# IamArmanNikkhah/viewport-entropy-toolkit

Hardware: NVIDIA B200
Metric: user-frame samples/sec (bin+weighted entropy, 200 tiles) (higher is better)
Workload: dtype f64

## Files before the change

### include/vet_b200.h

```cpp
#ifndef VET_B200_H
#define VET_B200_H

#include <stdint.h>

#ifdef __cplusplus
extern "C" {
#endif

typedef struct vet_handle vet_handle;

typedef enum {
  VET_OK = 0,
  VET_ERR_INVALID_ARG = -1,
  VET_ERR_CUDA = -2,
  VET_ERR_UNSUPPORTED = -3,
  VET_ERR_NOMEM = -4
} vet_status;

enum { VET_F32 = 0, VET_F64 = 1 };
enum { VET_TRANSITION_LITERAL = 0, VET_TRANSITION_TEXTBOOK = 1 };
enum { VET_MISSING = 0xFFFF };

enum {
  VET_FLAG_OUT_OF_RANGE = 1,
  VET_FLAG_EMPTY_FRAME = 2,
  VET_FLAG_NO_COMMON_USER = 4
};

typedef struct {
  int32_t device;
  int32_t video_width;
  int32_t video_height;
  int32_t num_tile_counts;
  const int32_t* tile_counts;
  double fov_angle;
  double power_factor;
  int32_t use_weight_distribution;
  const double* const* centres;
  const double* lon_by_px;
  const double* lat_by_py;
  const int32_t* num_tiles;
  int32_t naive_tile_width;
  int32_t naive_tile_height;
  int32_t regime;
} vet_config;

enum { VET_REGIME_AUTO = 0, VET_REGIME_DIRECT = 1 };

const char* vet_last_error(void);
const char* vet_version(void);

#define VET_I8_MIN_FRAMES 384
enum {
  VET_OPT_WEIGHTED_KERNEL = 0,
  VET_OPT_STREAM_KERNEL = 1,
  VET_OPT_TRANSITION_KERNEL = 2,
  VET_OPT_CLUSTER_TAIL = 3,
  VET_OPT_T3_PAIR_SCRATCH = 4,
  VET_OPT_T3_ASSUME_MISSING = 5,
  VET_OPT_ANALYZE_OVERLAP = 6,
  VET_OPT_HOST_BATCH_FRAMES = 7,
  VET_OPT_T4_LIST_CAP = 8,
  VET_OPT_CUDA_GRAPH = 9,
  VET_OPT_HOST_LAYOUT = 10,
  VET_OPT_COUNT = 11
};
int vet_set_option(vet_handle* h, int option, int value);
int vet_get_option(const vet_handle* h, int option, int* value);

int vet_create(vet_handle** out, const vet_config* cfg);
int vet_destroy(vet_handle* h);

int vet_num_tiles(const vet_handle* h, int k);
int64_t vet_num_cells(const vet_handle* h);

int vet_lattice(const vet_handle* h, int k, double* centres_host);
int vet_cell_lut(const vet_handle* h, int k, uint16_t* lut_host);

int vet_decode(vet_handle* h, const void* packed_dev, int dtype, int64_t n, double* vec_dev,
               int32_t* cell_dev, void* stream);

int vet_nearest_tile(vet_handle* h, int k, const double* vec_dev, int64_t n, int32_t* idx_dev,
                     void* stream);

int vet_tile_weights(vet_handle* h, int k, const double* vec_dev, int64_t n, double* w_dev,
                     void* stream);

int vet_angular_distances(vet_handle* h, int k, const double* vec_dev, int64_t n, double* d_dev,
                          void* stream);

int vet_vector_angles(vet_handle* h, const double* a_dev, const double* b_dev, int64_t n, double* d_dev,
                      void* stream);

int vet_spatial_vectors(vet_handle* h, const double* vec_dev, int64_t F, int64_t U,
                        double* entropy_dev, double* per_k_dev, double* hist0_dev,
                        uint16_t* assign0_dev, void* stream);

int vet_transition_vectors(vet_handle* h, const double* vec_dev, int64_t F, int64_t U,
                           double* entropy_dev, double* per_k_dev, int32_t* prev_count0_dev,
                           uint16_t* pairs0_dev, int mode, void* stream);

int vet_spatial(vet_handle* h, const void* packed_dev, int dtype, int64_t F, int64_t U,
                double* entropy_dev, double* per_k_dev, double* hist0_dev, uint16_t* assign0_dev,
                void* stream);

int vet_transition(vet_handle* h, const void* packed_dev, int dtype, int64_t F, int64_t U,
                   double* entropy_dev, double* per_k_dev, int32_t* prev_count0_dev,
                   uint16_t* pairs0_dev, int mode, void* stream);

int vet_analyze(vet_handle* h, const void* packed_dev, int dtype, int64_t F, int64_t U,
                double* sp_entropy_dev, double* sp_per_k_dev, double* hist0_dev, uint16_t* assign0_dev,
                double* tr_entropy_dev, double* tr_per_k_dev, int32_t* prev_count0_dev,
                uint16_t* pairs0_dev, int mode, void* stream);

int vet_spatial_host(vet_handle* h, const void* packed_host, int dtype, int64_t F, int64_t U,
                     double* entropy_host, double* per_k_host, double* hist0_host,
                     uint16_t* assign0_host);
int vet_transition_host(vet_handle* h, const void* packed_host, int dtype, int64_t F, int64_t U,
                        double* entropy_host, double* per_k_host, int32_t* prev_count0_host,
                        uint16_t* pairs0_host, int mode);
int vet_analyze_host(vet_handle* h, const void* packed_host, int dtype, int64_t F, int64_t U,
                     double* sp_entropy_host, double* sp_per_k_host, double* hist0_host, uint16_t* assign0_host,
                     double* tr_entropy_host, double* tr_per_k_host, int32_t* prev_count0_host,
                     uint16_t* pairs0_host, int mode);

int vet_users_accumulate(vet_handle* h, const void* packed_dev, int dtype, int64_t F, int64_t U,
                         int64_t total_frames, int64_t* acc_dev, void* stream);
int vet_users_finish(vet_handle* h, const int64_t* acc_dev, int64_t U, int64_t total_frames,
                     double* entropy_dev, double* per_k_dev, double* hist0_dev, void* stream);

int vet_naive_points(vet_handle* h, const double* lonlat_dev, int64_t F, int64_t U, int32_t tile_width,
                     int32_t tile_height, int32_t use_weight_distribution, double* entropy_dev,
                     int32_t* lon_idx_dev, int32_t* lat_idx_dev, void* stream);

int vet_poll_flags(vet_handle* h, void* stream, uint32_t* flags);

int64_t vet_launch_count(const vet_handle* h);
int64_t vet_graph_replays(const vet_handle* h);

enum {
  VET_KERNEL_STREAM = 0,
  VET_KERNEL_EPILOGUE = 1,
  VET_KERNEL_TRANSITION = 2,
  VET_KERNEL_TRANSITION_TAIL = 3,
  VET_KERNEL_COUNT = 4
};
int vet_profile_enable(vet_handle* h, int on);
int vet_profile_read(vet_handle* h, double* ms_by_kernel, int64_t* launches_by_kernel);

#ifdef __cplusplus
}
#endif
#endif
```

### viewport_entropy_toolkit_b200/_native.py

```python
from __future__ import annotations

import ctypes as C
import os
from pathlib import Path
from typing import Optional

LIB_PATH = Path(__file__).resolve().parent / "_lib" / "libvet_b200.so"

VET_OK = 0
VET_ERR_INVALID_ARG = -1
VET_ERR_CUDA = -2
VET_ERR_UNSUPPORTED = -3
VET_ERR_NOMEM = -4

VET_F32, VET_F64 = 0, 1
VET_TRANSITION_LITERAL, VET_TRANSITION_TEXTBOOK = 0, 1
VET_MISSING = 0xFFFF
VET_FLAG_OUT_OF_RANGE, VET_FLAG_EMPTY_FRAME, VET_FLAG_NO_COMMON_USER = 1, 2, 4
VET_REGIME_AUTO, VET_REGIME_DIRECT = 0, 1
I8_MIN_FRAMES = 384

OPTIONS = {
    "weighted_kernel": (0, {"auto": 0, "fp64": 1, "i8": 2}),
    "stream_kernel": (1, {"auto": 0, "simple": 1, "cells": 2, "global": 3}),
    "transition_kernel": (2, {"auto": 0, "v1": 1, "v2": 2, "v3": 3}),
    "cluster_tail": (3, {"off": 0, "auto": 1, "force": 2}),
    "t3_pair_scratch": (4, {"off": 0, "on": 1}),
    "t3_assume_missing": (5, {"off": 0, "on": 1}),
    "analyze_overlap": (6, {"off": 0, "on": 1}),
    "host_batch_frames": (7, {"auto": 0}),
    "t4_list_cap": (8, {"auto": 0}),
    "cuda_graph": (9, {"off": 0, "on": 1}),
    "host_layout": (10, {"tuv": 0, "uv": 1}),
}


class VetConfig(C.Structure):
    _fields_ = [
        ("device", C.c_int32),
        ("video_width", C.c_int32),
        ("video_height", C.c_int32),
        ("num_tile_counts", C.c_int32),
        ("tile_counts", C.POINTER(C.c_int32)),
        ("fov_angle", C.c_double),
        ("power_factor", C.c_double),
        ("use_weight_distribution", C.c_int32),
        ("centres", C.POINTER(C.POINTER(C.c_double))),
        ("lon_by_px", C.POINTER(C.c_double)),
        ("lat_by_py", C.POINTER(C.c_double)),
        ("num_tiles", C.POINTER(C.c_int32)),
        ("naive_tile_width", C.c_int32),
        ("naive_tile_height", C.c_int32),
        ("regime", C.c_int32),
    ]


_P = C.c_void_p
_I64 = C.c_int64
SYMBOLS = {
    "vet_last_error": (C.c_char_p, []),
    "vet_version": (C.c_char_p, []),
    "vet_set_option": (C.c_int, [_P, C.c_int, C.c_int]),
    "vet_get_option": (C.c_int, [_P, C.c_int, C.POINTER(C.c_int)]),
    "vet_create": (C.c_int, [C.POINTER(_P), C.POINTER(VetConfig)]),
    "vet_destroy": (C.c_int, [_P]),
    "vet_num_tiles": (C.c_int, [_P, C.c_int]),
    "vet_num_cells": (_I64, [_P]),
    "vet_lattice": (C.c_int, [_P, C.c_int, _P]),
    "vet_cell_lut": (C.c_int, [_P, C.c_int, _P]),
    "vet_decode": (C.c_int, [_P, _P, C.c_int, _I64, _P, _P, _P]),
    "vet_nearest_tile": (C.c_int, [_P, C.c_int, _P, _I64, _P, _P]),
    "vet_tile_weights": (C.c_int, [_P, C.c_int, _P, _I64, _P, _P]),
    "vet_angular_distances": (C.c_int, [_P, C.c_int, _P, _I64, _P, _P]),
    "vet_vector_angles": (C.c_int, [_P, _P, _P, _I64, _P, _P]),
    "vet_spatial_vectors": (C.c_int, [_P, _P, _I64, _I64, _P, _P, _P, _P, _P]),
    "vet_transition_vectors": (C.c_int, [_P, _P, _I64, _I64, _P, _P, _P, _P, C.c_int, _P]),
    "vet_spatial": (C.c_int, [_P, _P, C.c_int, _I64, _I64, _P, _P, _P, _P, _P]),
    "vet_transition": (C.c_int, [_P, _P, C.c_int, _I64, _I64, _P, _P, _P, _P, C.c_int, _P]),
    "vet_analyze": (C.c_int, [_P, _P, C.c_int, _I64, _I64, _P, _P, _P, _P, _P, _P, _P, _P, C.c_int, _P]),
    "vet_spatial_host": (C.c_int, [_P, _P, C.c_int, _I64, _I64, _P, _P, _P, _P]),
    "vet_transition_host": (C.c_int, [_P, _P, C.c_int, _I64, _I64, _P, _P, _P, _P, C.c_int]),
    "vet_analyze_host": (C.c_int, [_P, _P, C.c_int, _I64, _I64, _P, _P, _P, _P, _P, _P, _P, _P, C.c_int]),
    "vet_users_accumulate": (C.c_int, [_P, _P, C.c_int, _I64, _I64, _I64, _P, _P]),
    "vet_users_finish": (C.c_int, [_P, _P, _I64, _I64, _P, _P, _P, _P]),
    "vet_naive_points": (C.c_int, [_P, _P, _I64, _I64, C.c_int32, C.c_int32, C.c_int32, _P, _P, _P, _P]),
    "vet_poll_flags": (C.c_int, [_P, _P, C.POINTER(C.c_uint32)]),
    "vet_launch_count": (_I64, [_P]),
    "vet_graph_replays": (_I64, [_P]),
    "vet_profile_enable": (C.c_int, [_P, C.c_int]),
    "vet_profile_read": (C.c_int, [_P, C.POINTER(C.c_double), C.POINTER(C.c_int64)]),
}
KERNEL_NAMES = ("stream", "epilogue", "transition", "transition_tail")

_lib: Optional[C.CDLL] = None


class NativeLibraryError(RuntimeError):
    """The CUDA library is missing or incomplete (build it with
    `python __graft_entry__.py`)."""


def load_library() -> C.CDLL:
    global _lib
    if _lib is not None:
        return _lib
    path = Path(os.environ.get("VET_B200_LIB", LIB_PATH))
    if not path.exists():
        raise NativeLibraryError(
            f"{path} not found: the CUDA extension is not built (run `python __graft_entry__.py`); "
            "there is no CPU fallback")
    lib = C.CDLL(str(path))
    for name, (restype, argtypes) in SYMBOLS.items():
        try:
            fn = getattr(lib, name)
        except AttributeError as e:
            raise NativeLibraryError(f"{path} does not export {name}") from e
        fn.restype = restype
        fn.argtypes = argtypes
    _lib = lib
    return lib


def last_error() -> str:
    return load_library().vet_last_error().decode("utf-8", "replace")
```

### viewport_entropy_toolkit_b200/csrc/vet_whist_i8.cuh

```cuda
#pragma once
#include <cuda.h>

#include "vet_common.cuh"
#include "vet_stream_tma.cuh"

namespace vet {

constexpr int kI8Slices = 5;
constexpr int kI8FracBits = 39;
constexpr int kI8TilesPerBlock = 48;
constexpr int kI8N = kI8Slices * kI8TilesPerBlock;
constexpr int kI8M = 128;
constexpr int kI8BK = 128;
constexpr int kI8Stages = 3;
constexpr int kI8StagesOne = 4;
constexpr int kI8ABytes = kI8M * kI8BK;
constexpr int kI8BBytes = kI8N * kI8BK;
constexpr int kI8StageBytes = 2 * kI8ABytes + kI8BBytes;
constexpr int kI8Threads = 192;
constexpr int kI8MaxSplit = 8;
constexpr int kI8TmemCols = 512;
constexpr int kI8SmemBytes = kI8Stages * kI8StageBytes + 1024;
static_assert(kI8StageBytes % 1024 == 0 && (kI8ABytes + kI8BBytes) % 1024 == 0, "stages must keep the 1024 B swizzle alignment");
static_assert(kI8StagesOne * (kI8ABytes + kI8BBytes) <= kI8Stages * kI8StageBytes, "both layouts share one ring");

__device__ __forceinline__ void tma_load_2d(uint32_t dst, const void* tmap, uint32_t bar, int c0, int c1) {
  asm volatile(
      "cp.async.bulk.tensor.2d.shared::cluster.global.mbarrier::complete_tx::bytes [%0], [%1, {%3, %4}], [%2];" ::"r"(dst),
      "l"(tmap), "r"(bar), "r"(c0), "r"(c1)
      : "memory");
}
__device__ __forceinline__ void tc_fence_before() { asm volatile("tcgen05.fence::before_thread_sync;" ::: "memory"); }
__device__ __forceinline__ void tc_fence_after() { asm volatile("tcgen05.fence::after_thread_sync;" ::: "memory"); }
__device__ __forceinline__ void tc_alloc(uint32_t smem_dst, uint32_t cols) {
  asm volatile("tcgen05.alloc.cta_group::1.sync.aligned.shared::cta.b32 [%0], %1;" ::"r"(smem_dst), "r"(cols) : "memory");
  asm volatile("tcgen05.relinquish_alloc_permit.cta_group::1.sync.aligned;" ::: "memory");
}
__device__ __forceinline__ void tc_dealloc(uint32_t taddr, uint32_t cols) {
  asm volatile("tcgen05.dealloc.cta_group::1.sync.aligned.b32 %0, %1;" ::"r"(taddr), "r"(cols) : "memory");
}
__device__ __forceinline__ void tc_commit(uint32_t bar) {
  asm volatile("tcgen05.commit.cta_group::1.mbarrier::arrive::one.shared::cluster.b64 [%0];" ::"r"(bar) : "memory");
}
__device__ __forceinline__ void tc_mma_i8(uint32_t d, uint64_t adesc, uint64_t bdesc, uint32_t idesc, uint32_t accumulate) {
  asm volatile(
      "{\n"
      ".reg .pred p;\n"
      "setp.ne.b32 p, %4, 0;\n"
      "tcgen05.mma.cta_group::1.kind::i8 [%0], %1, %2, %3, p;\n"
      "}\n" ::"r"(d),
      "l"(adesc), "l"(bdesc), "r"(idesc), "r"(accumulate)
      : "memory");
}
__device__ __forceinline__ void tc_ld16(uint32_t taddr, uint32_t (&r)[16]) {
  asm volatile(
      "tcgen05.ld.sync.aligned.32x32b.x16.b32 {%0, %1, %2, %3, %4, %5, %6, %7, %8, %9, %10, %11, %12, %13, %14, %15}, [%16];"
      : "=r"(r[0]), "=r"(r[1]), "=r"(r[2]), "=r"(r[3]), "=r"(r[4]), "=r"(r[5]), "=r"(r[6]), "=r"(r[7]), "=r"(r[8]), "=r"(r[9]),
        "=r"(r[10]), "=r"(r[11]), "=r"(r[12]), "=r"(r[13]), "=r"(r[14]), "=r"(r[15])
      : "r"(taddr)
      : "memory");
}
__device__ __forceinline__ void tc_wait_ld() { asm volatile("tcgen05.wait::ld.sync.aligned;" ::: "memory"); }

__device__ __forceinline__ uint64_t i8_smem_desc(uint32_t saddr) {
  return (uint64_t)((saddr & 0x3FFFFu) >> 4) | (1ull << 16) | ((uint64_t)(1024 >> 4) << 32) | (1ull << 46) | (2ull << 61);
}
constexpr uint32_t kI8InstrDesc = (2u << 4) | ((uint32_t)(kI8N >> 3) << 17) | ((uint32_t)(kI8M >> 4) << 24);

struct WhistI8Args {
  int64_t F;
  int T;
  int n_blocks;
  int row_a;
  int row_b;
  const uint32_t* flag_b;
  const uint32_t* run_if;
  int shift;
  int accumulate;
  const int2* kb_range;
  double* hist;
  int ksplit;
  int* part;
};

__global__ void __launch_bounds__(kI8Threads, 1)
k_whist_i8(const __grid_constant__ CUtensorMap tm_cnt, const __grid_constant__ CUtensorMap tm_w, WhistI8Args a) {
  const int tile_id = blockIdx.x / a.ksplit;
  const int sp = blockIdx.x % a.ksplit;
  const int nb = tile_id % a.n_blocks;
  const int mb = tile_id / a.n_blocks;
  if (a.run_if && a.run_if[mb] == 0u) return;
  extern __shared__ unsigned char smem_dyn[];
  __shared__ __align__(8) unsigned long long s_full[kI8StagesOne], s_empty[kI8StagesOne], s_accum;
  __shared__ uint32_t s_tmem;
  const int warp = threadIdx.x >> 5, lane = threadIdx.x & 31;
  const uint32_t ring = (smem_u32(smem_dyn) + 1023u) & ~1023u;
  int2 kr = a.kb_range[nb];
  if (a.ksplit > 1) {
    const int per = (kr.y - kr.x + a.ksplit - 1) / a.ksplit;
    kr.x = min(kr.y, kr.x + sp * per);
    kr.y = min(kr.y, kr.x + per);
  }
  const bool two = a.flag_b && a.flag_b[mb] != 0u;

  const uint32_t nstages = two ? kI8Stages : kI8StagesOne;
  const uint32_t stage_bytes = two ? (uint32_t)kI8StageBytes : (uint32_t)(kI8ABytes + kI8BBytes);
  const uint32_t w_off = two ? 2u * kI8ABytes : (uint32_t)kI8ABytes;
  if (threadIdx.x == 0) {
    for (int i = 0; i < kI8StagesOne; ++i) {
      mbar_init(smem_u32(&s_full[i]), 1);
      mbar_init(smem_u32(&s_empty[i]), 1);
    }
    mbar_init(smem_u32(&s_accum), 1);
    asm volatile("fence.mbarrier_init.release.cluster;" ::: "memory");
  }
  if (warp == 1) tc_alloc(smem_u32(&s_tmem), kI8TmemCols);
  tc_fence_before();
  __syncthreads();
  tc_fence_after();
  const uint32_t tmem = s_tmem;

  if (warp == 0) {
    if (lane == 0) {
      uint32_t stage = 0, phase = 0;
      for (int kb = kr.x; kb < kr.y; ++kb) {
        mbar_wait(smem_u32(&s_empty[stage]), phase ^ 1u);
        const uint32_t bar = smem_u32(&s_full[stage]);
        const uint32_t base = ring + stage * stage_bytes;
        mbar_expect_tx(bar, stage_bytes);
        tma_load_2d(base, &tm_cnt, bar, kb * kI8BK, a.row_a + mb * kI8M);
        if (two) tma_load_2d(base + kI8ABytes, &tm_cnt, bar, kb * kI8BK, a.row_b + mb * kI8M);
        tma_load_2d(base + w_off, &tm_w, bar, kb * kI8BK, nb * kI8N);
        if (++stage == nstages) {
          stage = 0;
          phase ^= 1u;
        }
      }
    }
  } else if (warp == 1) {
    if (lane == 0) {
      uint32_t stage = 0, phase = 0;
      for (int kb = kr.x; kb < kr.y; ++kb) {
        mbar_wait(smem_u32(&s_full[stage]), phase);
        tc_fence_after();
        const uint32_t base = ring + stage * stage_bytes;
#pragma unroll
        for (int k = 0; k < kI8BK / 32; ++k) {
          const uint32_t acc = (kb > kr.x || k > 0) ? 1u : 0u;
          const uint64_t bdesc = i8_smem_desc(base + w_off + k * 32);
          tc_mma_i8(tmem, i8_smem_desc(base + k * 32), bdesc, kI8InstrDesc, acc);
          if (two) tc_mma_i8(tmem + 256, i8_smem_desc(base + kI8ABytes + k * 32), bdesc, kI8InstrDesc, acc);
        }
        tc_commit(smem_u32(&s_empty[stage]));
        if (++stage == nstages) {
          stage = 0;
          phase ^= 1u;
        }
      }
      tc_commit(smem_u32(&s_accum));
    }
    __syncwarp();
  } else {
    const int q = warp & 3;
    const int64_t f = (int64_t)mb * kI8M + q * 32 + lane;
    const uint32_t lane_base = tmem + ((uint32_t)(q * 32) << 16);
    if (a.ksplit > 1) {
      int* __restrict__ part = a.part + ((int64_t)tile_id * a.ksplit + sp) * (2 * kI8N * kI8M) + q * 32 + lane;
      const bool have = kr.y > kr.x;
      if (have) {
        mbar_wait(smem_u32(&s_accum), 0u);
        tc_fence_after();
      }
#pragma unroll 1
      for (int c0 = 0; c0 < kI8N; c0 += 16) {
        uint32_t r0[16], r1[16];
#pragma unroll
        for (int j = 0; j < 16; ++j) r0[j] = r1[j] = 0u;
        if (have) {
          tc_ld16(lane_base + c0, r0);
          if (two) tc_ld16(lane_base + 256 + c0, r1);
          tc_wait_ld();
        }
#pragma unroll
        for (int j = 0; j < 16; ++j) {
          __stcg(part + (c0 + j) * kI8M, (int)r0[j]);
          if (two) __stcg(part + (kI8N + c0 + j) * kI8M, (int)r1[j]);
        }
      }
    } else {
      mbar_wait(smem_u32(&s_accum), 0u);
      tc_fence_after();
#pragma unroll 1
      for (int j0 = 0; j0 < kI8TilesPerBlock; j0 += 16) {
        double v[16];
#pragma unroll
        for (int j = 0; j < 16; ++j) v[j] = 0.0;
#pragma unroll
        for (int s = kI8Slices - 1; s >= 0; --s) {
          uint32_t r0[16], r1[16];
          tc_ld16(lane_base + s * kI8TilesPerBlock + j0, r0);
          if (two) tc_ld16(lane_base + 256 + s * kI8TilesPerBlock + j0, r1);
          tc_wait_ld();
          const double scale = __longlong_as_double((long long)(1023 + 8 * s - kI8FracBits + a.shift) << 52);
#pragma unroll
          for (int j = 0; j < 16; ++j) {
            long long x = (long long)(int)r0[j];
            if (two) x += (long long)(int)r1[j] << 8;
            v[j] = fma((double)x, scale, v[j]);
          }
        }
        if (f < a.F) {
          double* __restrict__ row = a.hist + f * (int64_t)a.T;
#pragma unroll
          for (int j = 0; j < 16; ++j) {
            const int tile = nb * kI8TilesPerBlock + j0 + j;
            if (tile < a.T) row[tile] = a.accumulate ? row[tile] + v[j] : v[j];
          }
        }
      }
    }
  }
  tc_fence_before();
  __syncthreads();
  if (warp == 1) tc_dealloc(tmem, kI8TmemCols);
}

__global__ void __launch_bounds__(kI8M) k_whist_i8_finish(WhistI8Args a) {
  const int tile_id = blockIdx.y;
  const int nb = tile_id % a.n_blocks;
  const int mb = tile_id / a.n_blocks;
  if (a.run_if && a.run_if[mb] == 0u) return;
  const int j = blockIdx.x;
  const int tile = nb * kI8TilesPerBlock + j;
  const int64_t f = (int64_t)mb * kI8M + threadIdx.x;
  if (tile >= a.T || f >= a.F) return;
  const bool two = a.flag_b && a.flag_b[mb] != 0u;
  const int* __restrict__ part = a.part + (int64_t)tile_id * a.ksplit * (2 * kI8N * kI8M) + threadIdx.x;
  int x0[kI8Slices], x1[kI8Slices];
#pragma unroll
  for (int s = 0; s < kI8Slices; ++s) x0[s] = x1[s] = 0;
#pragma unroll
  for (int sp = 0; sp < kI8MaxSplit; ++sp) {
    if (sp < a.ksplit) {
#pragma unroll
      for (int s = 0; s < kI8Slices; ++s) {
        const int* p = part + (int64_t)sp * (2 * kI8N * kI8M) + (s * kI8TilesPerBlock + j) * kI8M;
        x0[s] += __ldcg(p);
        if (two) x1[s] += __ldcg(p + kI8N * kI8M);
      }
    }
  }
  double v = 0.0;
#pragma unroll
  for (int s = kI8Slices - 1; s >= 0; --s) {
    long long x = (long long)x0[s];
    if (two) x += (long long)x1[s] << 8;
    const double scale = __longlong_as_double((long long)(1023 + 8 * s - kI8FracBits + a.shift) << 52);
    v = fma((double)x, scale, v);
  }
  double* __restrict__ row = a.hist + f * (int64_t)a.T;
  row[tile] = a.accumulate ? row[tile] + v : v;
}

struct CntPlanesArgs {
  const uint32_t* cnt;
  int64_t F;
  int cpad;
  int kp;
  int64_t plane_stride;
  uint8_t* planes;
  uint8_t* dirty;
  uint32_t* hi1;
  uint32_t* hi2;
};

__global__ void __launch_bounds__(256) k_cnt_planes(CntPlanesArgs a) {
  const int lane = threadIdx.x & 31;
  const int64_t warp = (blockIdx.x * (int64_t)blockDim.x + threadIdx.x) >> 5;
  const int64_t nwarps = ((int64_t)gridDim.x * blockDim.x) >> 5;
  const int upr = a.kp >> 7;
  const int64_t units = a.F * upr;
  uint32_t* __restrict__ p0 = reinterpret_cast<uint32_t*>(a.planes);
  uint32_t* __restrict__ p1 = reinterpret_cast<uint32_t*>(a.planes + a.plane_stride);
  uint32_t* __restrict__ p2 = reinterpret_cast<uint32_t*>(a.planes + 2 * a.plane_stride);
  constexpr int kUnroll = 4;
  for (int64_t u0 = warp * kUnroll; u0 < units; u0 += nwarps * kUnroll) {
    uint4 v[kUnroll];
#pragma unroll
    for (int i = 0; i < kUnroll; ++i) {
      const int64_t u = u0 + i;
      v[i] = make_uint4(0u, 0u, 0u, 0u);
      if (u < units) {
        const int64_t f = u / upr;
        const int c = (int)(u % upr) * 128 + lane * 4;
        if (c < a.cpad) v[i] = __ldg(reinterpret_cast<const uint4*>(a.cnt + f * (int64_t)a.cpad + c));
      }
    }
#pragma unroll
    for (int i = 0; i < kUnroll; ++i) {
      const int64_t u = u0 + i;
      if (u < units) {
        const int64_t f = u / upr;
        const int64_t o = (f * (int64_t)a.kp + (u % upr) * 128) / 4 + lane;
        const uint32_t w1 = pack_bytes(v[i], 8), w2 = pack_bytes(v[i], 16);
        p0[o] = pack_bytes(v[i], 0);
        p1[o] = w1;
        p2[o] = w2;
        if (w1 && *reinterpret_cast<volatile uint32_t*>(&a.hi1[f >> 7]) == 0u) atomicOr(&a.hi1[f >> 7], 1u);
        if (w2 && *reinterpret_cast<volatile uint32_t*>(&a.hi2[f >> 7]) == 0u) atomicOr(&a.hi2[f >> 7], 1u);
        if (u % upr == 0 && lane == 0) a.dirty[f] = 3;
      }
    }
  }
}

}
```

Measured before the change: 418.2 billion.

## Restructure i8 weighted-histogram kernel with per-block k-lists, variable N, in-kernel third plane

Replaces the contiguous per-block k-range with an explicit list of k-blocks per tile block, makes the MMA N width and tiles-per-block runtime values, and interleaves slices per tile in the TMEM column layout. The third count plane (high bits) is now handled by a second sweep inside the same kernel, with a drain barrier to reuse TMEM, instead of a separate accumulate launch. The run_if early exit is removed. This aims to skip empty k-blocks and cut launches and hist read-modify-write passes, at the cost of a more complex barrier protocol and extra partial-buffer space.

```diff
diff --git a/include/vet_b200.h b/include/vet_b200.h
--- a/include/vet_b200.h
+++ b/include/vet_b200.h
@@ -63,7 +63,8 @@
   VET_OPT_T4_LIST_CAP = 8,
   VET_OPT_CUDA_GRAPH = 9,
   VET_OPT_HOST_LAYOUT = 10,
-  VET_OPT_COUNT = 11
+  VET_OPT_I8_LAYOUT = 11,
+  VET_OPT_COUNT = 12
 };
 int vet_set_option(vet_handle* h, int option, int value);
 int vet_get_option(const vet_handle* h, int option, int* value);
diff --git a/viewport_entropy_toolkit_b200/_native.py b/viewport_entropy_toolkit_b200/_native.py
--- a/viewport_entropy_toolkit_b200/_native.py
+++ b/viewport_entropy_toolkit_b200/_native.py
@@ -32,6 +32,7 @@
     "t4_list_cap": (8, {"auto": 0}),
     "cuda_graph": (9, {"off": 0, "on": 1}),
     "host_layout": (10, {"tuv": 0, "uv": 1}),
+    "i8_layout": (11, {"lists": 0, "hull": 1}),
 }
 
 
diff --git a/viewport_entropy_toolkit_b200/csrc/vet_whist_i8.cuh b/viewport_entropy_toolkit_b200/csrc/vet_whist_i8.cuh
--- a/viewport_entropy_toolkit_b200/csrc/vet_whist_i8.cuh
+++ b/viewport_entropy_toolkit_b200/csrc/vet_whist_i8.cuh
@@ -65,23 +65,30 @@
 __device__ __forceinline__ uint64_t i8_smem_desc(uint32_t saddr) {
   return (uint64_t)((saddr & 0x3FFFFu) >> 4) | (1ull << 16) | ((uint64_t)(1024 >> 4) << 32) | (1ull << 46) | (2ull << 61);
 }
-constexpr uint32_t kI8InstrDesc = (2u << 4) | ((uint32_t)(kI8N >> 3) << 17) | ((uint32_t)(kI8M >> 4) << 24);
+__device__ __forceinline__ uint32_t i8_instr_desc(int n) {
+  return (2u << 4) | ((uint32_t)(n >> 3) << 17) | ((uint32_t)(kI8M >> 4) << 24);
+}
 
 struct WhistI8Args {
   int64_t F;
   int T;
   int n_blocks;
+  int tb;
+  int n;
   int row_a;
   int row_b;
+  int row_c;
   const uint32_t* flag_b;
-  const uint32_t* run_if;
-  int shift;
-  int accumulate;
-  const int2* kb_range;
+  const uint32_t* flag_c;
+  const int* kb;
   double* hist;
   int ksplit;
   int* part;
 };
+
+__device__ __forceinline__ double i8_scale(int s, int shift) {
+  return __longlong_as_double((long long)(1023 + 8 * s - kI8FracBits + shift) << 52);
+}
 
 __global__ void __launch_bounds__(kI8Threads, 1)
 k_whist_i8(const __grid_constant__ CUtensorMap tm_cnt, const __grid_constant__ CUtensorMap tm_w, WhistI8Args a) {
@@ -89,22 +96,23 @@
   const int sp = blockIdx.x % a.ksplit;
   const int nb = tile_id % a.n_blocks;
   const int mb = tile_id / a.n_blocks;
-  if (a.run_if && a.run_if[mb] == 0u) return;
   extern __shared__ unsigned char smem_dyn[];
-  __shared__ __align__(8) unsigned long long s_full[kI8StagesOne], s_empty[kI8StagesOne], s_accum;
+  __shared__ __align__(8) unsigned long long s_full[kI8StagesOne], s_empty[kI8StagesOne], s_accum, s_drained;
   __shared__ uint32_t s_tmem;
   const int warp = threadIdx.x >> 5, lane = threadIdx.x & 31;
   const uint32_t ring = (smem_u32(smem_dyn) + 1023u) & ~1023u;
-  int2 kr = a.kb_range[nb];
+  int e0 = __ldg(a.kb + nb), e1 = __ldg(a.kb + nb + 1);
   if (a.ksplit > 1) {
-    const int per = (kr.y - kr.x + a.ksplit - 1) / a.ksplit;
-    kr.x = min(kr.y, kr.x + sp * per);
-    kr.y = min(kr.y, kr.x + per);
-  }
-  const bool two = a.flag_b && a.flag_b[mb] != 0u;
+    const int per = (e1 - e0 + a.ksplit - 1) / a.ksplit;
+    e0 = min(e1, e0 + sp * per);
+    e1 = min(e1, e0 + per);
+  }
+  const bool two = a.flag_b[mb] != 0u;
+  const bool third = a.flag_c[mb] != 0u;
 
   const uint32_t nstages = two ? kI8Stages : kI8StagesOne;
-  const uint32_t stage_bytes = two ? (uint32_t)kI8StageBytes : (uint32_t)(kI8ABytes + kI8BBytes);
+  const uint32_t b_bytes = (uint32_t)a.n * kI8BK;
+  const uint32_t stage_bytes = (two ? 2u * kI8ABytes : (uint32_t)kI8ABytes) + b_bytes;
   const uint32_t w_off = two ? 2u * kI8ABytes : (uint32_t)kI8ABytes;
   if (threadIdx.x == 0) {
     for (int i = 0; i < kI8StagesOne; ++i) {
@@ -112,6 +120,7 @@
       mbar_init(smem_u32(&s_empty[i]), 1);
     }
     mbar_init(smem_u32(&s_accum), 1);
+    mbar_init(smem_u32(&s_drained), 4 * 32);
     asm volatile("fence.mbarrier_init.release.cluster;" ::: "memory");
   }
   if (warp == 1) tc_alloc(smem_u32(&s_tmem), kI8TmemCols);
@@ -119,102 +128,124 @@
   __syncthreads();
   tc_fence_after();
   const uint32_t tmem = s_tmem;
+  const int sweeps = third ? 2 : 1;
 
   if (warp == 0) {
     if (lane == 0) {
       uint32_t stage = 0, phase = 0;
-      for (int kb = kr.x; kb < kr.y; ++kb) {
-        mbar_wait(smem_u32(&s_empty[stage]), phase ^ 1u);
-        const uint32_t bar = smem_u32(&s_full[stage]);
-        const uint32_t base = ring + stage * stage_bytes;
-        mbar_expect_tx(bar, stage_bytes);
-        tma_load_2d(base, &tm_cnt, bar, kb * kI8BK, a.row_a + mb * kI8M);
-        if (two) tma_load_2d(base + kI8ABytes, &tm_cnt, bar, kb * kI8BK, a.row_b + mb * kI8M);
-        tma_load_2d(base + w_off, &tm_w, bar, kb * kI8BK, nb * kI8N);
-        if (++stage == nstages) {
-          stage = 0;
-          phase ^= 1u;
+      for (int sw = 0; sw < sweeps; ++sw) {
+        const bool b = sw == 0 && two;
+        const uint32_t bytes = (b ? 2u * kI8ABytes : (uint32_t)kI8ABytes) + b_bytes;
+        const int row = (sw == 0 ? a.row_a : a.row_c) + mb * kI8M;
+        for (int e = e0; e < e1; ++e) {
+          const int kb = __ldg(a.kb + e);
+          mbar_wait(smem_u32(&s_empty[stage]), phase ^ 1u);
+          const uint32_t bar = smem_u32(&s_full[stage]);
+          const uint32_t base = ring + stage * stage_bytes;
+          mbar_expect_tx(bar, bytes);
+          tma_load_2d(base, &tm_cnt, bar, kb * kI8BK, row);
+          if (b) tma_load_2d(base + kI8ABytes, &tm_cnt, bar, kb * kI8BK, a.row_b + mb * kI8M);
+          tma_load_2d(base + w_off, &tm_w, bar, kb * kI8BK, nb * a.n);
+          if (++stage == nstages) {
+            stage = 0;
+            phase ^= 1u;
+          }
         }
       }
     }
   } else if (warp == 1) {
     if (lane == 0) {
       uint32_t stage = 0, phase = 0;
-      for (int kb = kr.x; kb < kr.y; ++kb) {
-        mbar_wait(smem_u32(&s_full[stage]), phase);
-        tc_fence_after();
-        const uint32_t base = ring + stage * stage_bytes;
-#pragma unroll
-        for (int k = 0; k < kI8BK / 32; ++k) {
-          const uint32_t acc = (kb > kr.x || k > 0) ? 1u : 0u;
-          const uint64_t bdesc = i8_smem_desc(base + w_off + k * 32);
-          tc_mma_i8(tmem, i8_smem_desc(base + k * 32), bdesc, kI8InstrDesc, acc);
-          if (two) tc_mma_i8(tmem + 256, i8_smem_desc(base + kI8ABytes + k * 32), bdesc, kI8InstrDesc, acc);
-        }
-        tc_commit(smem_u32(&s_empty[stage]));
-        if (++stage == nstages) {
-          stage = 0;
-          phase ^= 1u;
-        }
-      }
-      tc_commit(smem_u32(&s_accum));
+      const uint32_t idesc = i8_instr_desc(a.n);
+      for (int sw = 0; sw < sweeps; ++sw) {
+        const bool b = sw == 0 && two;
+        if (sw == 1) {
+          mbar_wait(smem_u32(&s_drained), 0u);
+          tc_fence_after();
+        }
+        for (int e = e0; e < e1; ++e) {
+          mbar_wait(smem_u32(&s_full[stage]), phase);
+          tc_fence_after();
+          const uint32_t base = ring + stage * stage_bytes;
+#pragma unroll
+          for (int k = 0; k < kI8BK / 32; ++k) {
+            const uint32_t acc = (e > e0 || k > 0) ? 1u : 0u;
+            const uint64_t bdesc = i8_smem_desc(base + w_off + k * 32);
+            tc_mma_i8(tmem, i8_smem_desc(base + k * 32), bdesc, idesc, acc);
+            if (b) tc_mma_i8(tmem + 256, i8_smem_desc(base + kI8ABytes + k * 32), bdesc, idesc, acc);
+          }
+          tc_commit(smem_u32(&s_empty[stage]));
+          if (++stage == nstages) {
+            stage = 0;
+            phase ^= 1u;
+          }
+        }
+        tc_commit(smem_u32(&s_accum));
+      }
     }
     __syncwarp();
   } else {
     const int q = warp & 3;
     const int64_t f = (int64_t)mb * kI8M + q * 32 + lane;
     const uint32_t lane_base = tmem + ((uint32_t)(q * 32) << 16);
-    if (a.ksplit > 1) {
-      int* __restrict__ part = a.part + ((int64_t)tile_id * a.ksplit + sp) * (2 * kI8N * kI8M) + q * 32 + lane;
-      const bool have = kr.y > kr.x;
+    const bool have = e1 > e0;
+    for (int sw = 0; sw < sweeps; ++sw) {
+      const bool b = sw == 0 && two;
+      if (sw == 1) {
+        tc_fence_before();
+        mbar_arrive(smem_u32(&s_drained));
+      }
       if (have) {
-        mbar_wait(smem_u32(&s_accum), 0u);
+        mbar_wait(smem_u32(&s_accum), (uint32_t)sw);
         tc_fence_after();
       }
+      if (a.ksplit > 1) {
+        int* __restrict__ part = a.part + ((int64_t)tile_id * a.ksplit + sp) * (3 * kI8N * kI8M) + q * 32 + lane;
+        if (sw == 1) part += 2 * kI8N * kI8M;
 #pragma unroll 1
-      for (int c0 = 0; c0 < kI8N; c0 += 16) {
-        uint32_t r0[16], r1[16];
-#pragma unroll
-        for (int j = 0; j < 16; ++j) r0[j] = r1[j] = 0u;
-        if (have) {
-          tc_ld16(lane_base + c0, r0);
-          if (two) tc_ld16(lane_base + 256 + c0, r1);
-          tc_wait_ld();
-        }
-#pragma unroll
-        for (int j = 0; j < 16; ++j) {
-          __stcg(part + (c0 + j) * kI8M, (int)r0[j]);
-          if (two) __stcg(part + (kI8N + c0 + j) * kI8M, (int)r1[j]);
-        }
-      }
-    } else {
-      mbar_wait(smem_u32(&s_accum), 0u);
-      tc_fence_after();
+        for (int c0 = 0; c0 < a.n; c0 += 16) {
+          uint32_t r0[16], r1[16];
+#pragma unroll
+          for (int j = 0; j < 16; ++j) r0[j] = r1[j] = 0u;
+          if (have) {
+            tc_ld16(lane_base + c0, r0);
+            if (b) tc_ld16(lane_base + 256 + c0, r1);
+            tc_wait_ld();
+          }
+#pragma unroll
+          for (int j = 0; j < 16; ++j) {
+            __stcg(part + (c0 + j) * kI8M, (int)r0[j]);
+            if (b) __stcg(part + (kI8N + c0 + j) * kI8M, (int)r1[j]);
+          }
+        }
+      } else {
+        const int shift = sw == 0 ? 0 : 16;
 #pragma unroll 1
-      for (int j0 = 0; j0 < kI8TilesPerBlock; j0 += 16) {
-        double v[16];
-#pragma unroll
-        for (int j = 0; j < 16; ++j) v[j] = 0.0;
-#pragma unroll
-        for (int s = kI8Slices - 1; s >= 0; --s) {
-          uint32_t r0[16], r1[16];
-          tc_ld16(lane_base + s * kI8TilesPerBlock + j0, r0);
-          if (two) tc_ld16(lane_base + 256 + s * kI8TilesPerBlock + j0, r1);
-          tc_wait_ld();
-          const double scale = __longlong_as_double((long long)(1023 + 8 * s - kI8FracBits + a.shift) << 52);
-#pragma unroll
-          for (int j = 0; j < 16; ++j) {
-            long long x = (long long)(int)r0[j];
-            if (two) x += (long long)(int)r1[j] << 8;
-            v[j] = fma((double)x, scale, v[j]);
-          }
-        }
-        if (f < a.F) {
-          double* __restrict__ row = a.hist + f * (int64_t)a.T;
-#pragma unroll
-          for (int j = 0; j < 16; ++j) {
-            const int tile = nb * kI8TilesPerBlock + j0 + j;
-            if (tile < a.T) row[tile] = a.accumulate ? row[tile] + v[j] : v[j];
+        for (int j0 = 0; j0 < a.tb; j0 += 16) {
+          double v[16];
+#pragma unroll
+          for (int j = 0; j < 16; ++j) v[j] = 0.0;
+#pragma unroll
+          for (int i = 0; i < kI8Slices; ++i) {
+            uint32_t r0[16], r1[16];
+            tc_ld16(lane_base + 5 * j0 + 16 * i, r0);
+            if (b) tc_ld16(lane_base + 256 + 5 * j0 + 16 * i, r1);
+            tc_wait_ld();
+#pragma unroll
+            for (int c = 0; c < 16; ++c) {
+              const int col = 16 * i + c, j = col / 5, sl = kI8Slices - 1 - col % 5;
+              long long x = (long long)(int)r0[c];
+              if (b) x += (long long)(int)r1[c] << 8;
+              v[j] = fma((double)x, i8_scale(sl, shift), v[j]);
+            }
+          }
+          if (f < a.F) {
+            double* __restrict__ row = a.hist + f * (int64_t)a.T;
+#pragma unroll
+            for (int j = 0; j < 16; ++j) {
+              const int tile = nb * a.tb + j0 + j;
+              if (j0 + j < a.tb && tile < a.T) row[tile] = sw == 1 ? row[tile] + v[j] : v[j];
+            }
           }
         }
       }
@@ -229,37 +260,37 @@
   const int tile_id = blockIdx.y;
   const int nb = tile_id % a.n_blocks;
   const int mb = tile_id / a.n_blocks;
-  if (a.run_if && a.run_if[mb] == 0u) return;
   const int j = blockIdx.x;
-  const int tile = nb * kI8TilesPerBlock + j;
+  const int tile = nb * a.tb + j;
   const int64_t f = (int64_t)mb * kI8M + threadIdx.x;
   if (tile >= a.T || f >= a.F) return;
-  const bool two = a.flag_b && a.flag_b[mb] != 0u;
-  const int* __restrict__ part = a.part + (int64_t)tile_id * a.ksplit * (2 * kI8N * kI8M) + threadIdx.x;
-  int x0[kI8Slices], x1[kI8Slices];
-#pragma unroll
-  for (int s = 0; s < kI8Slices; ++s) x0[s] = x1[s] = 0;
+  const bool two = a.flag_b[mb] != 0u;
+  const bool third = a.flag_c[mb] != 0u;
+  const int* __restrict__ part = a.part + (int64_t)tile_id * a.ksplit * (3 * kI8N * kI8M) + threadIdx.x;
+  int x0[kI8Slices], x1[kI8Slices], x2[kI8Slices];
+#pragma unroll
+  for (int s = 0; s < kI8Slices; ++s) x0[s] = x1[s] = x2[s] = 0;
 #pragma unroll
   for (int sp = 0; sp < kI8MaxSplit; ++sp) {
     if (sp < a.ksplit) {
 #pragma unroll
       for (int s = 0; s < kI8Slices; ++s) {
-        const int* p = part + (int64_t)sp * (2 * kI8N * kI8M) + (s * kI8TilesPerBlock + j) * kI8M;
+        const int* p = part + (int64_t)sp * (3 * kI8N * kI8M) + (5 * j + kI8Slices - 1 - s) * kI8M;
         x0[s] += __ldcg(p);
         if (two) x1[s] += __ldcg(p + kI8N * kI8M);
-      }
-    }
-  }
-  double v = 0.0;
+        if (third) x2[s] += __ldcg(p + 2 * kI8N * kI8M);
+      }
+    }
+  }
+  double v01 = 0.0, v2 = 0.0;
 #pragma unroll
   for (int s = kI8Slices - 1; s >= 0; --s) {
     long long x = (long long)x0[s];
     if (two) x += (long long)x1[s] << 8;
-    const double scale = __longlong_as_double((long long)(1023 + 8 * s - kI8FracBits + a.shift) << 52);
-    v = fma((double)x, scale, v);
-  }
-  double* __restrict__ row = a.hist + f * (int64_t)a.T;
-  row[tile] = a.accumulate ? row[tile] + v : v;
+    v01 = fma((double)x, i8_scale(s, 0), v01);
+    v2 = fma((double)x2[s], i8_scale(s, 16), v2);
+  }
+  a.hist[f * (int64_t)a.T + tile] = third ? v01 + v2 : v01;
 }
 
 struct CntPlanesArgs {
```

Measured after the change: 427.9 billion, median of 6. 1.02x the previous value.
